# khanhptnk/psketch

Measured on AMD Instinct MI355X. Metric: env-steps/sec (whole node), 12x12 craft_medium, batch=65536, higher is better.
Workload: dtype fp32; 1 GPU; craft_medium_12x12_w3_B65536_random_rollout_full_features_K32; world=craft_medium_12x12, envs_per_gpu=65536, global_batch=65536, window=3, n_features=404, obs_dtype=fp32, state_dtype=u8 (exact small integers; the reference's float64 arrays hold the same values), obs_ring=16, pool=1024, parallelism=env-shard x1, ticks_per_launch=32, launches=81, teach_table=auto, obs_store=sc1, tile=32, rollout_threads=512

## Files before the change

### psketch_amd/csrc/craft_episode.h

```cpp
#pragma once
#include "craft_device.h"

namespace craft {


__device__ __forceinline__ int hashed_action(const SimView& v, uint64_t seed, int64_t slot, int64_t tick) {
  const uint64_t gid = (uint64_t)(v.env_base + slot);
  return (int)((uint32_t)(splitmix64(seed ^ (gid << 20) ^ (uint64_t)tick) >> 32) % 6u);
}

__device__ __forceinline__ bool state_in_range(const SimView& v, const Agent& s) {
  return !(s.x < 1 || s.x > v.W - 2 || s.y < 1 || s.y > v.H - 2 || s.scen >= v.pool_count);
}

__device__ __forceinline__ void protocol_step(Agent& s, const int& act, const uint32_t& flags, int& d, int& counted, bool& restart) {
  if (s.frozen) {
    d = 1;
  } else {
    counted = 1;
    s.timer -= 1;
    d = (act == CRAFT_STOP) || s.timer <= 0;
    restart = d && (flags & CRAFT_STEP_AUTORESET);
  }
}

__device__ __forceinline__ void language_step_begin(const Agent& s, const int& act, int& d, int& counted, bool& bad) {
  if (s.frozen) {
    d = 1;
  } else {
    bad = act < 0 || act >= CRAFT_N_ACTIONS;
    counted = !bad;
  }
}
__device__ __forceinline__ void language_step_end(Agent& s, const int& act, int& d) {
  s.timer -= 1;
  d = (act == CRAFT_STOP) || s.timer <= 0;
  if (d) {
    s.frozen = 1;
    s.timer = max(s.timer, 0);
  }
}

__device__ __forceinline__ void restart_agent(Agent& s, uint32_t init_word, int maxT) {
  s.x = init_word & 0xff; s.y = (init_word >> 8) & 0xff; s.dir = (init_word >> 16) & 3;
  s.timer = maxT;
}

__device__ __forceinline__ int32_t queue_next(int32_t cur, const uint32_t& count, const uint32_t& step, const uint32_t& wrap) {
  if (cur < 0) return -1;
  uint32_t nx = (uint32_t)cur + step;
  if (nx >= count) {
    if (!wrap) return -1;
    nx -= count;
  }
  return (int32_t)nx;
}

__device__ __forceinline__ bool episode_ends(const Agent& s, int act) {
  return !s.frozen && (act == CRAFT_STOP || s.timer <= 1);
}

__device__ __forceinline__ bool language_episode_ends(const Agent& s, int act) {
  return !s.frozen && act >= 0 && act < CRAFT_N_ACTIONS && (act == CRAFT_STOP || s.timer <= 1);
}

__device__ __forceinline__ void restart_from_entry(Agent& s, const uint2& e, int maxT) {
  s.scen = (int)(e.x & 0xffffffu);
  s.task = (int)(e.x >> 24);
  restart_agent(s, e.y, maxT);
}

__device__ __forceinline__ uint32_t pose_word(const Agent& s) {
  return (uint32_t)s.x | ((uint32_t)s.y << 8) | ((uint32_t)s.dir << 16);
}

__device__ __forceinline__ int tape_action(const uint8_t* tape, const int& stride, int32_t cur, const Agent& s,
                                           const int& maxT) {
  const int p = maxT - s.timer;
  if (cur < 0 || p < 0 || p >= maxT) return CRAFT_STOP;
  return (int)tape[(int64_t)cur * stride + p];
}

template <int QB>
__device__ __forceinline__ void reload_grid_row(const uint4* pool_row, uint32_t* grid, const int& CS) {
  const int nchunk = CS >> 4;
#pragma unroll
  for (int b = 0; b < CRAFT_MAX_CELLS / 16; b += QB) {
    uint4 c[QB];
#pragma unroll
    for (int q = 0; q < QB; ++q)
      if (b + q < nchunk) c[q] = pool_row[b + q];
#pragma unroll
    for (int q = 0; q < QB; ++q)
      if (b + q < nchunk) {
        grid[4 * (b + q) + 0] = c[q].x; grid[4 * (b + q) + 1] = c[q].y;
        grid[4 * (b + q) + 2] = c[q].z; grid[4 * (b + q) + 3] = c[q].w;
      }
  }
}

__device__ __forceinline__ void freeze_agent(Agent& s) {
  s.frozen = 1;
  s.timer = max(s.timer, 0);
}

__device__ __forceinline__ int facing_cell(const Agent& s, int H) {
  return (s.x + dir_dx(s.dir)) * H + (s.y + dir_dy(s.dir));
}

__device__ __forceinline__ int satisfies_masked(const SimView& v, const uint8_t* g, const uint8_t* iv,
                                                const uint32_t (&m)[8], const Agent& s, uint32_t tt) {
  const int fc = facing_cell(s, v.H);
  uint32_t mw = 0;
#pragma unroll
  for (int w = 0; w < 8; ++w) mw |= (w == (fc >> 5)) ? m[w] : 0u;
  return satisfies_with(
      tt, [&](int arg) __attribute__((always_inline)) { return (int)iv[arg]; },
      [&]() __attribute__((always_inline)) { return ((mw >> (fc & 31)) & 1u) ? 0 : (int)g[fc]; });
}

__device__ __forceinline__ uint32_t agent_word(const Agent& s, bool live) {
  return live ? ((uint32_t)s.x | ((uint32_t)s.y << 8) | ((uint32_t)s.dir << 16) | (1u << 24)) : 0u;
}


__device__ __forceinline__ bool rewarded(const int& counted, const int& d, const int& succ) { return counted && d && succ == 1; }

template <class Args>
__device__ __forceinline__ void store_outputs(const Args& a, int64_t o, const int& d, const int& succ, const int& counted) {
  if (a.done) a.done[o] = (uint8_t)d;
  if (a.sat) a.sat[o] = (int8_t)succ;
  if (a.reward) a.reward[o] = rewarded(counted, d, succ) ? 1.0f : 0.0f;
}

__device__ __forceinline__ uint32_t pack_outputs(const int& d, const int& succ, const int& counted) {
  return (uint32_t)(uint8_t)d | ((uint32_t)(uint8_t)(int8_t)succ << 8) |
         ((uint32_t)rewarded(counted, d, succ) << 16) | (1u << 24);
}

__device__ __forceinline__ void tally_stats(const bool& live, const int& counted, const int& d, const int& succ,
                                            uint32_t& n_succ, uint32_t& n_end, uint32_t& n_step) {
  const uint64_t bs = __ballot(live && counted && d && succ == 1);
  const uint64_t be = __ballot(live && counted && d);
  const uint64_t bt = __ballot(live && counted);
  n_succ += (uint32_t)__popcll(bs);
  n_end += (uint32_t)__popcll(be);
  n_step += (uint32_t)__popcll(bt);
}
__device__ __forceinline__ void add_stats(const SimView& v, int64_t row, uint32_t n_succ, uint32_t n_end, uint32_t n_step) {
  unsigned long long* r = reinterpret_cast<unsigned long long*>(v.stats_part + 4 * row);
  atomicAdd(r + 0, (unsigned long long)n_succ);
  atomicAdd(r + 1, (unsigned long long)n_end);
  atomicAdd(r + 2, (unsigned long long)n_step);
}


template <class F>
__device__ __forceinline__ void for_each_masked_cell(const uint32_t (&m)[8], F f) {
#pragma unroll
  for (int w = 0; w < 8; ++w) {
    uint32_t mm = m[w];
    while (mm) {
      f(w * 32 + __ffs(mm) - 1);
      mm &= mm - 1;
    }
  }
}

__device__ __forceinline__ void apply_mask_to_row(const uint32_t (&m)[8], uint8_t* g) {
  for_each_masked_cell(m, [&](int c) __attribute__((always_inline)) { g[c] = 0; });
}


__device__ __forceinline__ void copy_row_words(uint32_t* dst, const uint32_t* src, const int& CS) {
  for (int q0 = 0; q0 < (CS >> 2); q0 += 12) {
    uint32_t w[12];
#pragma unroll
    for (int j = 0; j < 12; ++j) w[j] = q0 + j < (CS >> 2) ? src[q0 + j] : 0u;
#pragma unroll
    for (int j = 0; j < 12; ++j)
      if (q0 + j < (CS >> 2)) dst[q0 + j] = w[j];
  }
}

struct ClearList {
  uint32_t w = 0;
  __device__ __forceinline__ bool overflowed() const { return (w >> 31) != 0; }
  __device__ __forceinline__ uint32_t count() const { return (w >> 24) & 3; }
  __device__ __forceinline__ int cell(int i) const { return (int)((w >> (8 * i)) & 0xffu); }
  __device__ __forceinline__ bool has_room() const { return !overflowed() && count() < 3; }
  __device__ __forceinline__ void clear() { w = 0; }
  __device__ __forceinline__ void push(int c) {
    const uint32_t nc = count();
    w = overflowed() ? w
        : nc < 3 ? ((w & 0x00ffffffu) | ((uint32_t)c << (8 * nc)) | ((nc + 1) << 24)) : (1u << 31);
  }
  template <class K>
  __device__ __forceinline__ void restore(uint8_t* g, const uint32_t* pristine, const int& CS, K kind) const {
    if (overflowed()) {
      copy_row_words(reinterpret_cast<uint32_t*>(g), pristine, CS);
    } else {
      const int nc = (int)count();
#pragma unroll
      for (int i = 0; i < 3; ++i)
        if (i < nc) {
          const int c = cell(i);
          g[c] = kind(i, c);
        }
    }
  }
  __device__ __forceinline__ void restore(uint8_t* g, const uint32_t* pristine, const int& CS) const {
    const uint8_t* pr = reinterpret_cast<const uint8_t*>(pristine);
    restore(g, pristine, CS, [&](int, int c) __attribute__((always_inline)) { return pr[c]; });
  }
};

__device__ __forceinline__ void apply_mask_to_row(const uint32_t (&m)[8], uint8_t* g, ClearList& clr) {
  for_each_masked_cell(m, [&](int c) __attribute__((always_inline)) {
    g[c] = 0;
    clr.push(c);
  });
}

__device__ __forceinline__ void load_pool_row(const uint4* pool_row, uint32_t* pristine, uint32_t* grid, const int& CS) {
  const int nchunk = CS >> 4;
  for (int q0 = 0; q0 < nchunk; q0 += 4) {
    uint4 cq[4];
#pragma unroll
    for (int j = 0; j < 4; ++j)
      if (q0 + j < nchunk) cq[j] = pool_row[q0 + j];
#pragma unroll
    for (int j = 0; j < 4; ++j)
      if (q0 + j < nchunk) {
        const int q = 4 * (q0 + j);
        pristine[q + 0] = grid[q + 0] = cq[j].x;
        pristine[q + 1] = grid[q + 1] = cq[j].y;
        pristine[q + 2] = grid[q + 2] = cq[j].z;
        pristine[q + 3] = grid[q + 3] = cq[j].w;
      }
  }
}

__device__ __forceinline__ void cleared_mask(const uint32_t* pristine, const uint32_t* grid, const int& C, uint32_t (&m)[8]) {
#pragma unroll
  for (int i = 0; i < 8; ++i) m[i] = 0u;
#pragma unroll
  for (int q = 0; q < CRAFT_MAX_CELLS / 4; ++q)
    if (q < (C + 3) >> 2)
      m[q >> 3] |= byte_tops(nonzero_bytes(pristine[q]) & zero_bytes(grid[q])) << (4 * (q & 7));
}

__device__ __forceinline__ void publish_state(const SimView& v, const int64_t& slot, const uint64_t& st, const uint32_t* ivw,
                                              const uint32_t* m, bool sc1) {
  if (sc1) {
    typedef unsigned int u4v __attribute__((ext_vector_type(4)));
    const __amdgpu_buffer_rsrc_t inv_r = __builtin_amdgcn_make_buffer_rsrc(v.inv, 0, 0x7fffffff, 0x00020000);
    const __amdgpu_buffer_rsrc_t msk_r = __builtin_amdgcn_make_buffer_rsrc(v.mask, 0, 0x7fffffff, 0x00020000);
    const int off = (int)(slot * 32);
    __hip_atomic_store((gu64*)(v.state + slot), (unsigned long long)st, __ATOMIC_RELAXED,
                       __HIP_MEMORY_SCOPE_AGENT);
    __builtin_amdgcn_raw_buffer_store_b128(u4v{ivw[0], ivw[1], ivw[2], ivw[3]}, inv_r, off, 0, 16);
    __builtin_amdgcn_raw_buffer_store_b128(u4v{ivw[4], ivw[5], ivw[6], ivw[7]}, inv_r, off + 16, 0, 16);
    __builtin_amdgcn_raw_buffer_store_b128(u4v{m[0], m[1], m[2], m[3]}, msk_r, off, 0, 16);
    __builtin_amdgcn_raw_buffer_store_b128(u4v{m[4], m[5], m[6], m[7]}, msk_r, off + 16, 0, 16);
  } else {
    v.state[slot] = st;
    v.inv[2 * slot] = make_uint4(ivw[0], ivw[1], ivw[2], ivw[3]);
    v.inv[2 * slot + 1] = make_uint4(ivw[4], ivw[5], ivw[6], ivw[7]);
    v.mask[2 * slot] = make_uint4(m[0], m[1], m[2], m[3]);
    v.mask[2 * slot + 1] = make_uint4(m[4], m[5], m[6], m[7]);
  }
}

}
```

### psketch_amd/csrc/craft_rollout_split.h

```cpp
#pragma once
#include <type_traits>

#include "craft_episode.h"
#include "craft_obs.h"

namespace craft {

__host__ __device__ inline int split_stage_bytes(int tile, int CS) { return tile * (8 + 4 + 64) + tile * CS + tile * 40; }
__host__ __device__ inline int split_lds_bytes(int tile, int GS, int F, int CS, bool flat) {
  auto up16 = [](int x) { return (x + 15) & ~15; };
  return up16(3 * tile * GS) + 2 * up16(tile * F) + 2 * tile * kInvStride + 2 * tile * 4 +
         CRAFT_MAX_TASKS * 2 + CRAFT_MAX_RECIPES * 12 + 16 + 32 + 4 * tile * 4 +
         (flat ? split_stage_bytes(tile, CS) : 0);
}

template <int WIN, int TILE, int NT, int FMT, int WPE, bool GIVEN, bool FLAT = false, bool QUEUE = false,
          bool TAPE = false>
__global__ __launch_bounds__(NT, WPE) void rollout_split_kernel(SimView v, RolloutArgs a) {
  extern __shared__ __attribute__((aligned(16))) uint8_t smem[];
  static_assert(!(QUEUE && FLAT), "the queue variant runs work units, one per tile");
  static_assert(!TAPE || (QUEUE && !GIVEN), "the tape is the queue's: one row per entry");
  constexpr int DW = (WIN == 3 && TILE == 32 && NT == 512) ? 2 : 1;
  constexpr int E0 = 64 + 64 * DW;
  static_assert(NT >= E0 + 64 && TILE <= 64, "a producer, the scatter waves and at least one streaming wave");
  constexpr int P = 64 * DW / TILE;
  auto up16 = [](int x) { return (x + 15) & ~15; };
  const int GS = v.GS, F = v.F;
  const uint32_t rcv = v.rcw[min((int)(threadIdx.x & 63), CRAFT_MAX_RECIPES * 3 - 1)];
  uint8_t* s_grid = smem;
  uint8_t* s_pristine = smem + 2 * TILE * GS;
  const int obs_buf = up16(TILE * F);
  uint8_t* s_obs = smem + up16(3 * TILE * GS);
  uint8_t* s_inv = s_obs + 2 * obs_buf;
  uint32_t* s_agent = reinterpret_cast<uint32_t*>(s_inv + 2 * TILE * kInvStride);
  uint16_t* s_task = reinterpret_cast<uint16_t*>(s_agent + 2 * TILE);
  uint32_t* s_rc = reinterpret_cast<uint32_t*>(s_task + CRAFT_MAX_TASKS);
  uint32_t* s_ctrl = s_rc + CRAFT_MAX_RECIPES * 3;
  uint32_t* s_item = s_ctrl + 4;
  uint32_t* s_out = s_item + 8;
  uint8_t* s_stage = reinterpret_cast<uint8_t*>(s_out + 4 * TILE);

  const int tid = threadIdx.x;
  const int64_t n = v.n_envs;
  const bool want_obs = a.obs != nullptr;
  constexpr int esz = obs_elem_bytes(FMT);
  const int n_tiles = (int)((n + TILE - 1) / TILE);
  const int n_chunks = (a.n_ticks + a.chunk - 1) / a.chunk;
  const uint32_t n_units = (uint32_t)n_tiles * (uint32_t)n_chunks;

  Agent s{};
  uint64_t st = 0;
  uint32_t init_word = 0, task_word = 0;
  ClearList clr;
  ClearList clr_prev;
  uint32_t chg = 0;
  constexpr uint32_t kRestart = 0x80000000u;
  constexpr uint32_t kReload = 0x40000000u;
  int32_t cur = -1;
  uint2 qe = make_uint2(0u, 0u);
  int act_nx = CRAFT_STOP;
  int sync = 0;
  bool live = false;
  int64_t slot = 0;
  const uint32_t* pw = reinterpret_cast<const uint32_t*>(s_pristine + tid * GS);
  auto grid_of = [&](int p) __attribute__((always_inline)) { return s_grid + (p & 1) * TILE * GS + tid * GS; };
  auto inv_of = [&](int p) __attribute__((always_inline)) { return s_inv + (p & 1) * TILE * kInvStride + tid * kInvStride; };
  uint32_t n_succ = 0, n_end = 0, n_step = 0;

  auto tick_c = [&](int k, int p, bool lds_out) __attribute__((always_inline)) {
    const int64_t tick = a.tick0 + k;
    const int64_t r = tick % a.ring;
    int d = 0, succ = -1, counted = 0;
    uint8_t* g = grid_of(p);
    uint8_t* iv = inv_of(p);
    s = unpack_state(st);
    if (live) {
      if constexpr (QUEUE) {
        if (sync == 1 || chg == kReload)
          copy_row_words(reinterpret_cast<uint32_t*>(g), reinterpret_cast<const uint32_t*>(grid_of(p ^ 1)), v.CS);
        else if (chg) g[chg - 1] = 0;
      } else if (sync == 1) {
        copy_row_words(reinterpret_cast<uint32_t*>(g), reinterpret_cast<const uint32_t*>(grid_of(p ^ 1)), v.CS);
      } else if (sync == 2) {
        if (chg == kRestart) clr_prev.restore(g, pw, v.CS);
        else if (chg) g[chg - 1] = 0;
      }
      if (sync) {
        const uint32_t* src = reinterpret_cast<const uint32_t*>(inv_of(p ^ 1));
        uint32_t w[8];
#pragma unroll
        for (int i = 0; i < 8; ++i) w[i] = src[i];
#pragma unroll
        for (int i = 0; i < 8; ++i) reinterpret_cast<uint32_t*>(iv)[i] = w[i];
      }
      sync = sync ? 2 : 1;
      chg = 0;
      const int act = TAPE ? act_nx : GIVEN ? a.actions[(int64_t)k * n + slot] : hashed_action(v, a.seed, slot, tick);
      bool restart = false;
      protocol_step(s, act, a.flags, d, counted, restart);
      if (d) succ = satisfies(v, g, iv, s, task_word);
      int32_t ended = -1, epose = -1;
      if constexpr (QUEUE) {
        if (restart) {
          ended = cur;
          epose = (int32_t)pose_word(s);
          cur = queue_next(cur, a.q_count, a.q_step, a.q_wrap);
          if (cur >= 0) {
            restart_from_entry(s, qe, v.maxT);
            task_word = s_task[s.task];
            init_word = qe.y;
#pragma unroll
            for (int w = 0; w < 8; ++w) reinterpret_cast<uint32_t*>(iv)[w] = 0u;
            load_pool_row(reinterpret_cast<const uint4*>(v.pool + (size_t)s.scen * v.CS),
                          reinterpret_cast<uint32_t*>(s_pristine + tid * GS), reinterpret_cast<uint32_t*>(g), v.CS);
            chg = kReload;
            const int32_t nxt = queue_next(cur, a.q_count, a.q_step, a.q_wrap);
            if (nxt >= 0) qe = a.q_entries[nxt];
          } else {
            freeze_agent(s);
          }
        }
      } else if (restart) {
        restart_agent(s, init_word, v.maxT);
#pragma unroll
        for (int w = 0; w < 8; ++w) reinterpret_cast<uint32_t*>(iv)[w] = 0u;
        clr.restore(g, pw, v.CS);
        clr_prev = clr;
        clr.clear();
        chg = kRestart;
      } else if (d && !s.frozen) {
        freeze_agent(s);
      }
      if (!d) {
        bool inv_changed = false, mask_changed = false;
        uint32_t m_unused[8] = {0, 0, 0, 0, 0, 0, 0, 0};
        const int fc = facing_cell(s, v.H);
        if (act < 0 || act >= CRAFT_N_ACTIONS) latch_error(v.err, CRAFT_EBADACTION, slot);
        else transition<true>(v, s_rc, g, iv, s, m_unused, act, inv_changed, mask_changed, rcv, slot);
        if (mask_changed) {
          chg = 1u + (uint32_t)fc;
          if constexpr (!QUEUE) clr.push(fc);
        }
      }
      st = pack_state(s);
      if (lds_out) s_out[(p & 3) * TILE + tid] = pack_outputs(d, succ, counted);
      else store_outputs(a, r * n + slot, d, succ, counted);
      if constexpr (QUEUE) {
        if (a.ep_end) a.ep_end[r * n + slot] = ended;
        if (a.end_pose) a.end_pose[r * n + slot] = epose;
        if (a.ep_now) a.ep_now[r * n + slot] = s.frozen ? -1 : cur;
      }
      if constexpr (TAPE) {
        act_nx = tape_action(a.tape, a.tape_stride, cur, s, v.maxT);
        if (a.step_now) a.step_now[r * n + slot] = s.frozen ? -1 : v.maxT - s.timer;
        if (a.act_next) a.act_next[r * n + slot] = s.frozen ? -1 : act_nx;
      }
    } else if (lds_out && tid < TILE) {
      s_out[(p & 3) * TILE + tid] = 0u;
    }
    tally_stats(live, counted, d, succ, n_succ, n_end, n_step);
    s_agent[(p & 1) * TILE + tid] = agent_word(s, live);
  };

  uint64_t* sg_state = reinterpret_cast<uint64_t*>(s_stage);
  uint32_t* sg_init = reinterpret_cast<uint32_t*>(s_stage + TILE * 8);
  uint4* sg_inv = reinterpret_cast<uint4*>(s_stage + TILE * 12);
  uint4* sg_mask = reinterpret_cast<uint4*>(s_stage + TILE * 44);
  uint8_t* sg_pool = s_stage + TILE * 76;
  uint64_t* ob_state = reinterpret_cast<uint64_t*>(sg_pool + TILE * v.CS);
  uint32_t* ob_mask = reinterpret_cast<uint32_t*>(ob_state + TILE);

  auto load_tile = [&](int t, int p, auto STAGED) __attribute__((always_inline)) {
    constexpr bool staged = decltype(STAGED)::value;
    const int64_t env0 = (int64_t)t * TILE;
    const int nE = (int)min((int64_t)TILE, n - env0);
    slot = env0 + tid;
    live = tid < nE;
    uint32_t m[8] = {0, 0, 0, 0, 0, 0, 0, 0};
    uint32_t ivr[8] = {0, 0, 0, 0, 0, 0, 0, 0};
    if (live) {
      uint4 i0, i1, m0, m1;
      if constexpr (staged) {
        st = sg_state[tid];
        init_word = sg_init[tid];
        i0 = sg_inv[2 * tid]; i1 = sg_inv[2 * tid + 1];
        m0 = sg_mask[2 * tid]; m1 = sg_mask[2 * tid + 1];
      } else {
        st = v.state[slot];
        init_word = v.init[slot];
        if constexpr (QUEUE) cur = a.q_cursor[slot];
        i0 = v.inv[2 * slot]; i1 = v.inv[2 * slot + 1];
        m0 = v.mask[2 * slot]; m1 = v.mask[2 * slot + 1];
        if constexpr (QUEUE) {
          const int32_t nxt = queue_next(cur, a.q_count, a.q_step, a.q_wrap);
          if (nxt >= 0) qe = a.q_entries[nxt];
        }
      }
      ivr[0] = i0.x; ivr[1] = i0.y; ivr[2] = i0.z; ivr[3] = i0.w;
      ivr[4] = i1.x; ivr[5] = i1.y; ivr[6] = i1.z; ivr[7] = i1.w;
      m[0] = m0.x; m[1] = m0.y; m[2] = m0.z; m[3] = m0.w;
      m[4] = m1.x; m[5] = m1.y; m[6] = m1.z; m[7] = m1.w;
      s = unpack_state(st);
      if (!state_in_range(v, s)) {
        latch_error(v.err, CRAFT_EINVAL, slot);
        live = false;
      }
      if constexpr (TAPE) act_nx = tape_action(a.tape, a.tape_stride, cur, s, v.maxT);
    }
    chg = 0;
    clr.clear();
    clr_prev.clear();
    sync = 0;
    if (live) {
      task_word = s_task[s.task];
      uint32_t* g0 = reinterpret_cast<uint32_t*>(grid_of(p));
      uint32_t* pwm = reinterpret_cast<uint32_t*>(s_pristine + tid * GS);
      const uint4* gsrc = reinterpret_cast<const uint4*>(v.pool + (size_t)s.scen * v.CS);
      const uint4* lsrc = reinterpret_cast<const uint4*>(sg_pool + tid * v.CS);
      const int nchunk = v.CS >> 4;
      if constexpr (staged) {
        for (int q0 = 0; q0 < nchunk; ++q0) {
          const uint4 c = lsrc[q0];
          const int q = 4 * q0;
          pwm[q + 0] = g0[q + 0] = c.x;
          pwm[q + 1] = g0[q + 1] = c.y;
          pwm[q + 2] = g0[q + 2] = c.z;
          pwm[q + 3] = g0[q + 3] = c.w;
        }
      } else {
        load_pool_row(gsrc, pwm, g0, v.CS);
      }
      uint32_t* iv0 = reinterpret_cast<uint32_t*>(inv_of(p));
#pragma unroll
      for (int i = 0; i < 8; ++i) iv0[i] = ivr[i];
      apply_mask_to_row(m, grid_of(p), clr);
    }
    __builtin_amdgcn_fence(__ATOMIC_RELEASE, "wavefront");
    __builtin_amdgcn_wave_barrier();
    __builtin_amdgcn_fence(__ATOMIC_ACQUIRE, "wavefront");
  };

  auto publish = [&](int p, bool sc1) __attribute__((always_inline)) {
    uint32_t m[8];
    cleared_mask(pw, reinterpret_cast<const uint32_t*>(grid_of(p)), v.C, m);
    publish_state(v, slot, st, reinterpret_cast<const uint32_t*>(inv_of(p)), m, sc1);
    if constexpr (QUEUE) {
      v.init[slot] = init_word;
      a.q_cursor[slot] = cur;
    }
  };

  auto scatter_d = [&](int p, int nE) __attribute__((always_inline)) {
    const int l = tid - 64, e = l % TILE;
    const uint32_t ag = s_agent[(p & 1) * TILE + e];
    if (e < nE && ag)
      scatter_env_part<WIN, P>(v, s_grid + (p & 1) * TILE * GS + e * GS,
                               s_inv + (p & 1) * TILE * kInvStride + e * kInvStride, ag,
                               s_obs + (p & 1) * obs_buf + e * F, l / TILE);
  };

  auto stream_e = [&](int p, int t, int k, bool outs) __attribute__((always_inline)) {
    const int64_t env0 = (int64_t)t * TILE;
    const int nE = (int)min((int64_t)TILE, n - env0);
    const int64_t r = (a.tick0 + k) % a.ring;
    if (outs && tid - E0 < nE) {
      const uint32_t w = s_out[(p & 3) * TILE + tid - E0];
      if (w >> 24) {
        const int64_t o = r * n + env0 + (tid - E0);
        if (a.done) a.done[o] = (uint8_t)(w & 0xffu);
        if (a.sat) a.sat[o] = (int8_t)((w >> 8) & 0xffu);
        if (a.reward) a.reward[o] = ((w >> 16) & 1u) ? 1.0f : 0.0f;
      }
    }
    void* out = static_cast<uint8_t*>(a.obs) + r * n * (int64_t)F * esz;
    stream_obs<FMT, NT - E0, true>(s_obs + (p & 1) * obs_buf, out, env0, F, nE, v.obs_policy, tid - E0);
  };

  for (int t = tid; t < v.n_tasks; t += NT) s_task[t] = v.task_tab[t];
  for (int t = tid; t < CRAFT_MAX_RECIPES * 3; t += NT) s_rc[t] = v.rcw[t];
  if (want_obs) {
    uint4* z = reinterpret_cast<uint4*>(s_obs);
    for (int i = tid; i < (2 * obs_buf >> 4); i += NT) z[i] = make_uint4(0, 0, 0, 0);
  }

  if constexpr (FLAT) {
#ifdef CRAFT_STAMPS
    unsigned long long t_beg = __builtin_amdgcn_s_memrealtime();
#define SPLIT_NOW() __builtin_amdgcn_s_memrealtime()
#else
#define SPLIT_NOW() 0ull
#endif
    unsigned long long acc_work = 0, acc_wait = 0, acc_sw = 0, acc_pub = 0, acc_vm = 0, acc_ld = 0, acc_dma = 0;
    int cur_t = -1, cur_k = 0;
    bool staged = false;
    auto stage_state = [&](int t2) __attribute__((always_inline)) {
      const int64_t e0 = (int64_t)t2 * TILE;
      const int l = tid;
      typedef __attribute__((address_space(1))) void* gp;
      typedef __attribute__((address_space(3))) void* lp;
      if (l < TILE / 2) __builtin_amdgcn_global_load_lds((gp)(v.state + e0 + 2 * l), (lp)sg_state, 16, 0, 0);
      if (l < TILE / 4) __builtin_amdgcn_global_load_lds((gp)(v.init + e0 + 4 * l), (lp)sg_init, 16, 0, 0);
#pragma unroll
      for (int h = 0; h < 2 * TILE; h += 64) {
        __builtin_amdgcn_global_load_lds((gp)(v.inv + 2 * e0 + h + l), (lp)(sg_inv + h), 16, 0, 0);
        __builtin_amdgcn_global_load_lds((gp)(v.mask + 2 * e0 + h + l), (lp)(sg_mask + h), 16, 0, 0);
      }
    };
    auto stage_pool = [&]() __attribute__((always_inline)) {
      typedef __attribute__((address_space(1))) void* gp;
      typedef __attribute__((address_space(3))) void* lp;
      const int per = v.CS >> 4;
      int e = tid / per, c = tid - (tid / per) * per;
      const int de = 64 / per, dc = 64 - (64 / per) * per;
      for (int f0 = 0; f0 < TILE * per; f0 += 64) {
        const int f = f0 + tid;
        if (f < TILE * per) {
          const int scen = (int)((sg_state[e] >> 32) & 0xffffffu) % max(1, v.pool_count);
          __builtin_amdgcn_global_load_lds((gp)(v.pool + (size_t)scen * v.CS + 16 * c), (lp)(sg_pool + 16 * f0),
                                           16, 0, 0);
        }
        e += de;
        c += dc;
        if (c >= per) { c -= per; ++e; }
      }
    };
    auto fetch_now = [&]() __attribute__((always_inline)) -> int {
      unsigned long long r = 0;
      if (tid == 0) r = atomicAdd(a.queue, 1ull);
      const uint32_t d = (uint32_t)__builtin_amdgcn_readfirstlane((int)(uint32_t)r) - (uint32_t)a.qbase;
      return d < (uint32_t)n_tiles ? (int)d : -1;
    };
    const int K = a.n_ticks;
    const int kF = max(0, K - 6), kA = max(0, K - 4), kB = max(0, K - 3);
    uint32_t pend = 0;
    int64_t pub_slot = -1;
    int t_next = -1;
    auto produce = [&](int j) __attribute__((always_inline)) {
      if (cur_t != -2 && (cur_t < 0 || cur_k == K)) {
        const unsigned long long s0 = SPLIT_NOW();
        const int t = cur_t == -1 ? fetch_now() : t_next;
        if (staged) asm volatile("s_waitcnt vmcnt(0)" ::: "memory");
        const unsigned long long s1 = SPLIT_NOW();
        const bool pub = cur_t >= 0 && tid < TILE && live;
        const int64_t pslot = slot;
        if (pub) {
          uint32_t m[8];
          cleared_mask(pw, reinterpret_cast<const uint32_t*>(grid_of(j - 1)), v.C, m);
          ob_state[tid] = st;
#pragma unroll
          for (int i = 0; i < 8; ++i) ob_mask[8 * tid + i] = m[i];
        }
        const unsigned long long s2 = SPLIT_NOW();
        if (t >= 0) {
          cur_t = t;
          cur_k = 0;
          if (tid < TILE) {
            if (staged) load_tile(t, j & 1, std::true_type{});
            else load_tile(t, j & 1, std::false_type{});
          }
        } else {
          cur_t = -2;
        }
        staged = false;
        t_next = -1;
        pub_slot = pub ? pslot : -1;
        const unsigned long long s3 = SPLIT_NOW();
        acc_sw += s3 - s0;
        acc_vm += s1 - s0;
        acc_pub += s2 - s1;
        acc_ld += s3 - s2;
      }
      const bool have = cur_t >= 0;
      if (have) {
        const unsigned long long d0 = SPLIT_NOW();
        if (cur_k == kF && tid == 0) pend = (uint32_t)atomicAdd(a.queue, 1ull);
        if (cur_k == kA) {
          const uint32_t d = (uint32_t)__builtin_amdgcn_readfirstlane((int)pend) - (uint32_t)a.qbase;
          t_next = d < (uint32_t)n_tiles ? (int)d : -1;
          if (t_next >= 0 && (int64_t)(t_next + 1) * TILE <= n) {
            asm volatile("s_waitcnt lgkmcnt(0)" ::: "memory");
            stage_state(t_next);
          }
        }
        if (cur_k == kB && t_next >= 0 && (int64_t)(t_next + 1) * TILE <= n) {
          asm volatile("s_waitcnt vmcnt(0)" ::: "memory");
          stage_pool();
          staged = true;
        }
        acc_dma += SPLIT_NOW() - d0;
      }
      if (have && tid < TILE) tick_c(cur_k, j, true);
      if (pub_slot >= 0) {
        publish_state(v, pub_slot, ob_state[tid], reinterpret_cast<const uint32_t*>(inv_of(j - 1)), ob_mask + 8 * tid, false);
        pub_slot = -1;
      }
      if (tid == 0) {
        s_item[2 * (j & 3)] = have ? (uint32_t)cur_t + 1u : 0u;
        s_item[2 * (j & 3) + 1] = (uint32_t)cur_k;
      }
      if (have) ++cur_k;
    };
    auto interval_end = [&](int i, unsigned long long w0) __attribute__((always_inline)) -> bool {
      const unsigned long long w1 = SPLIT_NOW();
      asm volatile("s_waitcnt lgkmcnt(0)" ::: "memory");
      __builtin_amdgcn_s_barrier();
      asm volatile("" ::: "memory");
      acc_work += w1 - w0;
      acc_wait += SPLIT_NOW() - w1;
      return s_item[2 * (i & 3)] == 0;
    };
    if (tid < 64) {
      produce(0);
      asm volatile("s_waitcnt lgkmcnt(0)" ::: "memory");
      __builtin_amdgcn_s_barrier();
      asm volatile("" ::: "memory");
      for (int i = 0;; ++i) {
        const unsigned long long w0 = SPLIT_NOW();
        produce(i + 1);
        if (interval_end(i, w0)) break;
      }
    } else if (tid < E0) {
      asm volatile("s_waitcnt lgkmcnt(0)" ::: "memory");
      __builtin_amdgcn_s_barrier();
      asm volatile("" ::: "memory");
      for (int i = 0;; ++i) {
        const unsigned long long w0 = SPLIT_NOW();
        const uint32_t t1 = s_item[2 * (i & 3)];
        if (t1) scatter_d(i & 1, (int)min((int64_t)TILE, n - (int64_t)(t1 - 1) * TILE));
        if (interval_end(i, w0)) break;
      }
    } else {
      asm volatile("s_waitcnt lgkmcnt(0)" ::: "memory");
      __builtin_amdgcn_s_barrier();
      asm volatile("" ::: "memory");
      for (int i = 0;; ++i) {
        const unsigned long long w0 = SPLIT_NOW();
        if (i >= 1) {
          const uint32_t t1 = s_item[2 * ((i - 1) & 3)];
          if (t1) stream_e(i - 1, (int)t1 - 1, (int)s_item[2 * ((i - 1) & 3) + 1], true);
        }
        if (interval_end(i, w0)) break;
      }
    }
#ifdef CRAFT_STAMPS
    if (v.stamps) {
      uint64_t* row = v.stamps + 16 * (int64_t)blockIdx.x;
      if (tid == 0) {
        row[0] = t_beg; row[1] = acc_work; row[2] = acc_wait; row[6] = SPLIT_NOW(); row[7] = acc_sw;
        row[8] = acc_vm; row[9] = acc_pub; row[10] = acc_ld; row[11] = acc_dma;
      } else if (tid == 64) {
        row[3] = acc_work; row[4] = acc_wait;
      } else if (tid == E0) {
        row[5] = acc_work;
      }
    }
#endif
    (void)acc_work;
    (void)acc_wait;
    (void)acc_sw;
    (void)acc_pub;
    (void)acc_vm;
    (void)acc_ld;
    (void)acc_dma;
#undef SPLIT_NOW
  } else {
    (void)s_out;
    (void)s_stage;
#ifdef CRAFT_STAMPS
    uint64_t* srow_t = v.stamps ? v.stamps + 16 * (int64_t)blockIdx.x : nullptr;
    if (tid == 0 && srow_t) srow_t[0] = __builtin_amdgcn_s_memrealtime();
    int n_done = 0;
#endif
    bool first = (uint32_t)blockIdx.x < n_units;
    for (;;) {
      if (tid == 0)
        s_ctrl[0] = first ? (uint32_t)blockIdx.x
                          : (uint32_t)(gridDim.x + (atomicAdd(a.queue + 1, 1ull) - a.qbase1));
      first = false;
      __syncthreads();
      const uint32_t u = s_ctrl[0];
#ifdef CRAFT_STAMPS
      if (tid == 0 && srow_t && n_done < 12) srow_t[1 + n_done] = __builtin_amdgcn_s_memrealtime();
#endif
      if (u >= n_units) break;
      const int t = (int)(u % (uint32_t)n_tiles), c = (int)(u / (uint32_t)n_tiles);
      const int k0 = c * a.chunk, k1 = min(a.n_ticks, k0 + a.chunk);
      const int nq = k1 - k0;
      const int64_t env0 = (int64_t)t * TILE;
      const int nE = (int)min((int64_t)TILE, n - env0);

      const bool state_only = a.ring >= a.n_ticks;
      const bool handoff = c + 1 < n_chunks;
      auto full_release = [&]() __attribute__((always_inline)) {
        asm volatile("s_waitcnt vmcnt(0)" ::: "memory");
        __syncthreads();
        if (tid == 0) {
          __builtin_amdgcn_fence(__ATOMIC_RELEASE, "agent");
          asm volatile("s_waitcnt vmcnt(0)" ::: "memory");
          __hip_atomic_store((gu32*)(a.tile_done + t), (uint32_t)(c + 1), __ATOMIC_RELAXED,
                             __HIP_MEMORY_SCOPE_AGENT);
        }
      };
      if (tid < 64) {
        if (c > 0) {
          bool ok = true;
          if (tid == 0) {
            const gu32* f = (const gu32*)(a.tile_done + t);
            for (uint32_t spins = 0; __hip_atomic_load(f, __ATOMIC_RELAXED, __HIP_MEMORY_SCOPE_AGENT) < (uint32_t)c;) {
              __builtin_amdgcn_s_sleep(2);
              if (++spins > (1u << 26)) { ok = false; break; }
            }
            if (!ok) latch_error(v.err, CRAFT_EINVARIANT, env0);
          }
          __builtin_amdgcn_fence(__ATOMIC_ACQUIRE, "agent");
        }
        if (tid < TILE) {
          load_tile(t, 0, std::false_type{});
          tick_c(k0, 0, false);
        }
        if (want_obs) {
          __syncthreads();
          for (int i = 0; i <= nq; ++i) {
            if (tid < TILE && i + 1 < nq) tick_c(k0 + i + 1, i + 1, false);
            __syncthreads();
          }
        } else if (tid < TILE) {
          for (int q = 1; q < nq; ++q) tick_c(k0 + q, q, false);
        }
        if (tid < TILE && live) publish(nq - 1, handoff && state_only);
        if (handoff && state_only) {
          asm volatile("s_waitcnt vmcnt(0)" ::: "memory");
          if (tid == 0)
            __hip_atomic_store((gu32*)(a.tile_done + t), (uint32_t)(c + 1), __ATOMIC_RELAXED,
                               __HIP_MEMORY_SCOPE_AGENT);
        } else if (handoff) {
          full_release();
        }
      } else {
        if (want_obs) {
          __syncthreads();
          if (tid < E0) {
#pragma unroll 1
            for (int i = 0; i <= nq; ++i) {
              if (i < nq) scatter_d(i, nE);
              __syncthreads();
            }
          } else {
            for (int i = 0; i <= nq; ++i) {
              if (i >= 1) stream_e(i - 1, t, k0 + i - 1, false);
#ifdef CRAFT_STAMPS
              if (tid == E0 && srow_t && n_done == 0 && i == 1) srow_t[13] = __builtin_amdgcn_s_memrealtime();
#endif
              __syncthreads();
            }
          }
        }
        if (handoff && !state_only) full_release();
      }
      __syncthreads();
#ifdef CRAFT_STAMPS
      ++n_done;
#endif
    }
#ifdef CRAFT_STAMPS
    if (tid == 0 && srow_t) {
      srow_t[14] = (uint64_t)n_done;
      srow_t[15] = __builtin_amdgcn_s_memrealtime();
    }
#endif
  }

  if (tid == 0) add_stats(v, (int64_t)blockIdx.x, n_succ, n_end, n_step);
}

}
```

Before: 3.612 billion env-steps/s.

## Seed both grid buffers at tile load and drop per-tick row copy in rollout

At tile load the pool row and inventory are now written into both double-buffered LDS grid slots, with the same mask applied to each. That lets the non-flat path skip the full row copy on the first synced tick and apply only the single changed cell or the restart restore. The per-tick 64-bit modulo for the ring index is replaced by an incrementing ring counter, lds_out becomes a compile-time constant, and the overflow row copy uses 16-byte chunks. Optional timing stamps are added behind a macro. The cost is a larger initial LDS write per tile.

```diff
diff --git a/psketch_amd/csrc/craft_episode.h b/psketch_amd/csrc/craft_episode.h
--- a/psketch_amd/csrc/craft_episode.h
+++ b/psketch_amd/csrc/craft_episode.h
@@ -180,6 +180,26 @@
 #pragma unroll
     for (int j = 0; j < 12; ++j)
       if (q0 + j < (CS >> 2)) dst[q0 + j] = w[j];
+  }
+}
+
+__device__ __forceinline__ void copy_row_chunks(uint32_t* dst, const uint32_t* src, const int& CS) {
+  const int nchunk = CS >> 4;
+#pragma unroll 1
+  for (int c0 = 0; c0 < nchunk; c0 += 3) {
+    uint32_t w[12];
+#pragma unroll
+    for (int j = 0; j < 3; ++j)
+      if (c0 + j < nchunk) {
+#pragma unroll
+        for (int q = 0; q < 4; ++q) w[4 * j + q] = src[4 * (c0 + j) + q];
+      }
+#pragma unroll
+    for (int j = 0; j < 3; ++j)
+      if (c0 + j < nchunk) {
+#pragma unroll
+        for (int q = 0; q < 4; ++q) dst[4 * (c0 + j) + q] = w[4 * j + q];
+      }
   }
 }
 
@@ -197,17 +217,18 @@
   }
   template <class K>
   __device__ __forceinline__ void restore(uint8_t* g, const uint32_t* pristine, const int& CS, K kind) const {
-    if (overflowed()) {
-      copy_row_words(reinterpret_cast<uint32_t*>(g), pristine, CS);
-    } else {
-      const int nc = (int)count();
-#pragma unroll
-      for (int i = 0; i < 3; ++i)
-        if (i < nc) {
-          const int c = cell(i);
-          g[c] = kind(i, c);
-        }
-    }
+    if (overflowed()) copy_row_words(reinterpret_cast<uint32_t*>(g), pristine, CS);
+    else restore_listed(g, kind);
+  }
+  template <class K>
+  __device__ __forceinline__ void restore_listed(uint8_t* g, K kind) const {
+    const int nc = (int)count();
+#pragma unroll
+    for (int i = 0; i < 3; ++i)
+      if (i < nc) {
+        const int c = cell(i);
+        g[c] = kind(i, c);
+      }
   }
   __device__ __forceinline__ void restore(uint8_t* g, const uint32_t* pristine, const int& CS) const {
     const uint8_t* pr = reinterpret_cast<const uint8_t*>(pristine);
@@ -222,7 +243,8 @@
   });
 }
 
-__device__ __forceinline__ void load_pool_row(const uint4* pool_row, uint32_t* pristine, uint32_t* grid, const int& CS) {
+__device__ __forceinline__ void load_pool_row(const uint4* pool_row, uint32_t* pristine, uint32_t* grid, const int& CS,
+                                              uint32_t* grid2 = nullptr) {
   const int nchunk = CS >> 4;
   for (int q0 = 0; q0 < nchunk; q0 += 4) {
     uint4 cq[4];
@@ -237,6 +259,10 @@
         pristine[q + 1] = grid[q + 1] = cq[j].y;
         pristine[q + 2] = grid[q + 2] = cq[j].z;
         pristine[q + 3] = grid[q + 3] = cq[j].w;
+        if (grid2) {
+          grid2[q + 0] = cq[j].x; grid2[q + 1] = cq[j].y;
+          grid2[q + 2] = cq[j].z; grid2[q + 3] = cq[j].w;
+        }
       }
   }
 }
diff --git a/psketch_amd/csrc/craft_rollout_split.h b/psketch_amd/csrc/craft_rollout_split.h
--- a/psketch_amd/csrc/craft_rollout_split.h
+++ b/psketch_amd/csrc/craft_rollout_split.h
@@ -3,6 +3,10 @@
 
 #include "craft_episode.h"
 #include "craft_obs.h"
+
+#if defined(CRAFT_STAMPS) && defined(CRAFT_STAMPS_C)
+#define SPLIT_C_STAMPS 1
+#endif
 
 namespace craft {
 
@@ -67,38 +71,78 @@
   auto inv_of = [&](int p) __attribute__((always_inline)) { return s_inv + (p & 1) * TILE * kInvStride + tid * kInvStride; };
   uint32_t n_succ = 0, n_end = 0, n_step = 0;
 
-  auto tick_c = [&](int k, int p, bool lds_out) __attribute__((always_inline)) {
+#ifdef SPLIT_C_STAMPS
+  uint32_t c_acc[8] = {0, 0, 0, 0, 0, 0, 0, 0};
+  uint32_t c_last = 0;
+#define C_MARK(q)                                                          \
+  do {                                                                     \
+    if constexpr (!FLAT) {                                                 \
+      const uint32_t now_ = (uint32_t)__builtin_amdgcn_s_memrealtime();    \
+      c_acc[q] += now_ - c_last;                                           \
+      c_last = now_;                                                       \
+    }                                                                      \
+  } while (0)
+#define C_PIN(x) asm volatile("" : "+v"(x))
+#else
+#define C_MARK(q) do {} while (0)
+#define C_PIN(x) do {} while (0)
+#endif
+
+  auto restore_row = [&](const ClearList& c, uint8_t* g) __attribute__((always_inline)) {
+    if (c.overflowed()) {
+      copy_row_chunks(reinterpret_cast<uint32_t*>(g), pw, v.CS);
+    } else {
+      const uint8_t* pr = reinterpret_cast<const uint8_t*>(pw);
+      c.restore_listed(g, [&](int, int cell) __attribute__((always_inline)) { return pr[cell]; });
+    }
+  };
+
+  auto tick_c = [&](int k, int p, int r) __attribute__((always_inline)) {
+    constexpr bool lds_out = FLAT;
     const int64_t tick = a.tick0 + k;
-    const int64_t r = tick % a.ring;
     int d = 0, succ = -1, counted = 0;
     uint8_t* g = grid_of(p);
     uint8_t* iv = inv_of(p);
     s = unpack_state(st);
     if (live) {
-      if constexpr (QUEUE) {
-        if (sync == 1 || chg == kReload)
-          copy_row_words(reinterpret_cast<uint32_t*>(g), reinterpret_cast<const uint32_t*>(grid_of(p ^ 1)), v.CS);
-        else if (chg) g[chg - 1] = 0;
-      } else if (sync == 1) {
-        copy_row_words(reinterpret_cast<uint32_t*>(g), reinterpret_cast<const uint32_t*>(grid_of(p ^ 1)), v.CS);
-      } else if (sync == 2) {
-        if (chg == kRestart) clr_prev.restore(g, pw, v.CS);
-        else if (chg) g[chg - 1] = 0;
-      }
-      if (sync) {
+      auto copy_inv = [&]() __attribute__((always_inline)) {
         const uint32_t* src = reinterpret_cast<const uint32_t*>(inv_of(p ^ 1));
         uint32_t w[8];
 #pragma unroll
         for (int i = 0; i < 8; ++i) w[i] = src[i];
 #pragma unroll
         for (int i = 0; i < 8; ++i) reinterpret_cast<uint32_t*>(iv)[i] = w[i];
-      }
-      sync = sync ? 2 : 1;
+      };
+      if constexpr (!FLAT) {
+        if constexpr (QUEUE) {
+          if (chg == kReload)
+            copy_row_chunks(reinterpret_cast<uint32_t*>(g), reinterpret_cast<const uint32_t*>(grid_of(p ^ 1)), v.CS);
+          else if (chg) g[chg - 1] = 0;
+        } else {
+          if (chg == kRestart) restore_row(clr_prev, g);
+          else if (chg) g[chg - 1] = 0;
+        }
+        copy_inv();
+      } else {
+        if (sync == 1) {
+          copy_row_chunks(reinterpret_cast<uint32_t*>(g), reinterpret_cast<const uint32_t*>(grid_of(p ^ 1)), v.CS);
+        } else if (sync == 2) {
+          if (chg == kRestart) restore_row(clr_prev, g);
+          else if (chg) g[chg - 1] = 0;
+        }
+        if (sync) copy_inv();
+        sync = sync ? 2 : 1;
+      }
       chg = 0;
-      const int act = TAPE ? act_nx : GIVEN ? a.actions[(int64_t)k * n + slot] : hashed_action(v, a.seed, slot, tick);
+      C_MARK(0);
+      int act = TAPE ? act_nx : GIVEN ? a.actions[(int64_t)k * n + slot] : hashed_action(v, a.seed, slot, tick);
+      C_PIN(act);
+      C_MARK(1);
       bool restart = false;
       protocol_step(s, act, a.flags, d, counted, restart);
       if (d) succ = satisfies(v, g, iv, s, task_word);
+      C_PIN(succ);
+      C_MARK(2);
       int32_t ended = -1, epose = -1;
       if constexpr (QUEUE) {
         if (restart) {
@@ -124,13 +168,14 @@
         restart_agent(s, init_word, v.maxT);
 #pragma unroll
         for (int w = 0; w < 8; ++w) reinterpret_cast<uint32_t*>(iv)[w] = 0u;
-        clr.restore(g, pw, v.CS);
+        restore_row(clr, g);
         clr_prev = clr;
         clr.clear();
         chg = kRestart;
       } else if (d && !s.frozen) {
         freeze_agent(s);
       }
+      C_MARK(3);
       if (!d) {
         bool inv_changed = false, mask_changed = false;
         uint32_t m_unused[8] = {0, 0, 0, 0, 0, 0, 0, 0};
@@ -142,24 +187,27 @@
           if constexpr (!QUEUE) clr.push(fc);
         }
       }
+      C_PIN(s.x);
+      C_MARK(4);
       st = pack_state(s);
-      if (lds_out) s_out[(p & 3) * TILE + tid] = pack_outputs(d, succ, counted);
-      else store_outputs(a, r * n + slot, d, succ, counted);
+      if constexpr (lds_out) s_out[(p & 3) * TILE + tid] = pack_outputs(d, succ, counted);
+      else store_outputs(a, (int64_t)r * n + slot, d, succ, counted);
       if constexpr (QUEUE) {
-        if (a.ep_end) a.ep_end[r * n + slot] = ended;
-        if (a.end_pose) a.end_pose[r * n + slot] = epose;
-        if (a.ep_now) a.ep_now[r * n + slot] = s.frozen ? -1 : cur;
+        if (a.ep_end) a.ep_end[(int64_t)r * n + slot] = ended;
+        if (a.end_pose) a.end_pose[(int64_t)r * n + slot] = epose;
+        if (a.ep_now) a.ep_now[(int64_t)r * n + slot] = s.frozen ? -1 : cur;
       }
       if constexpr (TAPE) {
         act_nx = tape_action(a.tape, a.tape_stride, cur, s, v.maxT);
-        if (a.step_now) a.step_now[r * n + slot] = s.frozen ? -1 : v.maxT - s.timer;
-        if (a.act_next) a.act_next[r * n + slot] = s.frozen ? -1 : act_nx;
-      }
-    } else if (lds_out && tid < TILE) {
+        if (a.step_now) a.step_now[(int64_t)r * n + slot] = s.frozen ? -1 : v.maxT - s.timer;
+        if (a.act_next) a.act_next[(int64_t)r * n + slot] = s.frozen ? -1 : act_nx;
+      }
+    } else if constexpr (lds_out) {
       s_out[(p & 3) * TILE + tid] = 0u;
     }
     tally_stats(live, counted, d, succ, n_succ, n_end, n_step);
     s_agent[(p & 1) * TILE + tid] = agent_word(s, live);
+    C_MARK(5);
   };
 
   uint64_t* sg_state = reinterpret_cast<uint64_t*>(s_stage);
@@ -228,12 +276,18 @@
           pwm[q + 3] = g0[q + 3] = c.w;
         }
       } else {
-        load_pool_row(gsrc, pwm, g0, v.CS);
+        load_pool_row(gsrc, pwm, g0, v.CS, FLAT ? nullptr : reinterpret_cast<uint32_t*>(grid_of(p ^ 1)));
       }
       uint32_t* iv0 = reinterpret_cast<uint32_t*>(inv_of(p));
 #pragma unroll
       for (int i = 0; i < 8; ++i) iv0[i] = ivr[i];
       apply_mask_to_row(m, grid_of(p), clr);
+      if constexpr (!FLAT) {
+        uint32_t* iv1 = reinterpret_cast<uint32_t*>(inv_of(p ^ 1));
+#pragma unroll
+        for (int i = 0; i < 8; ++i) iv1[i] = ivr[i];
+        apply_mask_to_row(m, grid_of(p ^ 1));
+      }
     }
     __builtin_amdgcn_fence(__ATOMIC_RELEASE, "wavefront");
     __builtin_amdgcn_wave_barrier();
@@ -259,20 +313,19 @@
                                s_obs + (p & 1) * obs_buf + e * F, l / TILE);
   };
 
-  auto stream_e = [&](int p, int t, int k, bool outs) __attribute__((always_inline)) {
+  auto stream_e = [&](int p, int t, int r) __attribute__((always_inline)) {
     const int64_t env0 = (int64_t)t * TILE;
     const int nE = (int)min((int64_t)TILE, n - env0);
-    const int64_t r = (a.tick0 + k) % a.ring;
-    if (outs && tid - E0 < nE) {
+    if (FLAT && tid - E0 < nE) {
       const uint32_t w = s_out[(p & 3) * TILE + tid - E0];
       if (w >> 24) {
-        const int64_t o = r * n + env0 + (tid - E0);
+        const int64_t o = (int64_t)r * n + env0 + (tid - E0);
         if (a.done) a.done[o] = (uint8_t)(w & 0xffu);
         if (a.sat) a.sat[o] = (int8_t)((w >> 8) & 0xffu);
         if (a.reward) a.reward[o] = ((w >> 16) & 1u) ? 1.0f : 0.0f;
       }
     }
-    void* out = static_cast<uint8_t*>(a.obs) + r * n * (int64_t)F * esz;
+    void* out = static_cast<uint8_t*>(a.obs) + (int64_t)r * n * (int64_t)F * esz;
     stream_obs<FMT, NT - E0, true>(s_obs + (p & 1) * obs_buf, out, env0, F, nE, v.obs_policy, tid - E0);
   };
 
@@ -389,7 +442,7 @@
         }
         acc_dma += SPLIT_NOW() - d0;
       }
-      if (have && tid < TILE) tick_c(cur_k, j, true);
+      if (have && tid < TILE) tick_c(cur_k, j, 0);
       if (pub_slot >= 0) {
         publish_state(v, pub_slot, ob_state[tid], reinterpret_cast<const uint32_t*>(inv_of(j - 1)), ob_mask + 8 * tid, false);
         pub_slot = -1;
@@ -437,7 +490,7 @@
         const unsigned long long w0 = SPLIT_NOW();
         if (i >= 1) {
           const uint32_t t1 = s_item[2 * ((i - 1) & 3)];
-          if (t1) stream_e(i - 1, (int)t1 - 1, (int)s_item[2 * ((i - 1) & 3) + 1], true);
+          if (t1) stream_e(i - 1, (int)t1 - 1, (int)((a.tick0 + (int)s_item[2 * ((i - 1) & 3) + 1]) % a.ring));
         }
         if (interval_end(i, w0)) break;
       }
@@ -468,7 +521,9 @@
     (void)s_stage;
 #ifdef CRAFT_STAMPS
     uint64_t* srow_t = v.stamps ? v.stamps + 16 * (int64_t)blockIdx.x : nullptr;
+#ifndef SPLIT_C_STAMPS
     if (tid == 0 && srow_t) srow_t[0] = __builtin_amdgcn_s_memrealtime();
+#endif
     int n_done = 0;
 #endif
     bool first = (uint32_t)blockIdx.x < n_units;
@@ -479,7 +534,7 @@
       first = false;
       __syncthreads();
       const uint32_t u = s_ctrl[0];
-#ifdef CRAFT_STAMPS
+#if defined(CRAFT_STAMPS) && !defined(SPLIT_C_STAMPS)
       if (tid == 0 && srow_t && n_done < 12) srow_t[1 + n_done] = __builtin_amdgcn_s_memrealtime();
 #endif
       if (u >= n_units) break;
@@ -488,6 +543,8 @@
       const int nq = k1 - k0;
       const int64_t env0 = (int64_t)t * TILE;
       const int nE = (int)min((int64_t)TILE, n - env0);
+      const int r0 = (int)((a.tick0 + k0) % a.ring);
+      auto ring_next = [&](int r) __attribute__((always_inline)) { return r + 1 == a.ring ? 0 : r + 1; };
 
       const bool state_only = a.ring >= a.n_ticks;
       const bool handoff = c + 1 < n_chunks;
@@ -514,18 +571,38 @@
           }
           __builtin_amdgcn_fence(__ATOMIC_ACQUIRE, "agent");
         }
-        if (tid < TILE) {
-          load_tile(t, 0, std::false_type{});
-          tick_c(k0, 0, false);
-        }
+        if (tid < TILE) load_tile(t, 0, std::false_type{});
+        int rc = r0;
+#ifdef SPLIT_C_STAMPS
+        for (int q = 0; q < 8; ++q) c_acc[q] = 0;
+        c_last = (uint32_t)__builtin_amdgcn_s_memrealtime();
+#endif
         if (want_obs) {
-          __syncthreads();
-          for (int i = 0; i <= nq; ++i) {
-            if (tid < TILE && i + 1 < nq) tick_c(k0 + i + 1, i + 1, false);
+#pragma unroll 1
+          for (int i = -1; i <= nq; ++i) {
+            if (tid < TILE && i + 1 < nq) {
+              tick_c(k0 + i + 1, i + 1, rc);
+              rc = ring_next(rc);
+            }
             __syncthreads();
+#ifdef SPLIT_C_STAMPS
+            C_MARK(6);
+            c_acc[7] += 1;
+#endif
           }
+#ifdef SPLIT_C_STAMPS
+          if (tid == 0 && srow_t)
+            for (int q = 0; q < 8; ++q) {
+              srow_t[q] += c_acc[q];
+              srow_t[8 + q] = c_acc[q];
+            }
+#endif
         } else if (tid < TILE) {
-          for (int q = 1; q < nq; ++q) tick_c(k0 + q, q, false);
+#pragma unroll 1
+          for (int q = 0; q < nq; ++q) {
+            tick_c(k0 + q, q, rc);
+            rc = ring_next(rc);
+          }
         }
         if (tid < TILE && live) publish(nq - 1, handoff && state_only);
         if (handoff && state_only) {
@@ -546,9 +623,13 @@
               __syncthreads();
             }
           } else {
+            int re = r0;
             for (int i = 0; i <= nq; ++i) {
-              if (i >= 1) stream_e(i - 1, t, k0 + i - 1, false);
-#ifdef CRAFT_STAMPS
+              if (i >= 1) {
+                stream_e(i - 1, t, re);
+                re = ring_next(re);
+              }
+#if defined(CRAFT_STAMPS) && !defined(SPLIT_C_STAMPS)
               if (tid == E0 && srow_t && n_done == 0 && i == 1) srow_t[13] = __builtin_amdgcn_s_memrealtime();
 #endif
               __syncthreads();
@@ -562,13 +643,15 @@
       ++n_done;
 #endif
     }
-#ifdef CRAFT_STAMPS
+#if defined(CRAFT_STAMPS) && !defined(SPLIT_C_STAMPS)
     if (tid == 0 && srow_t) {
       srow_t[14] = (uint64_t)n_done;
       srow_t[15] = __builtin_amdgcn_s_memrealtime();
     }
 #endif
   }
+#undef C_MARK
+#undef C_PIN
 
   if (tid == 0) add_stats(v, (int64_t)blockIdx.x, n_succ, n_end, n_step);
 }
```

Result: no change. 3.609 billion env-steps/s (-0.1%).
